# stijnherfst/BrickMap

Hardware: AMD Instinct MI355X
Metric: Mrays/sec (primary x spp x bounces) at 1080p 4-bounce (higher is better)
Workload: dtype f32

## Files before the change

### brickmap_amd/csrc/device_types.h

```cpp
#pragma once
#include <cstddef>
#include <cstdint>

#if defined(__HIPCC__)
#define BM_VHD __host__ __device__ inline
#else
#define BM_VHD inline
#endif

namespace bm {

constexpr uint32_t kIndexBits = 0x00000FFFu;
constexpr uint32_t kLoadedBit = 0x80000000u;

BM_VHD uint32_t supercell_of(int sg_xy, int sg_xy2, int cx, int cy, int cz) {
	return static_cast<uint32_t>((cx >> 4) + (cy >> 4) * sg_xy + (cz >> 4) * sg_xy2);
}
BM_VHD size_t index_word_at(int sg_xy, int sg_xy2, int cx, int cy, int cz) {
	return static_cast<size_t>(supercell_of(sg_xy, sg_xy2, cx, cy, cz)) * 4096 + (cx & 15) + (cy & 15) * 16 + (cz & 15) * 256;
}
BM_VHD uint32_t cell_local_index(int cx, int cy, int cz) { return static_cast<uint32_t>(index_word_at(0, 0, cx & 15, cy & 15, cz & 15)); }
BM_VHD size_t brick_first_word(uint32_t pool_base_value, uint32_t index_word) {
	return (static_cast<size_t>(pool_base_value) + (index_word & kIndexBits)) << 4;
}
// ... 6 lines not shown
	int cf_shift;
	uint32_t cf_pxy;
	uint32_t cf_plane;
	uint32_t cf_magic;
	int cf_magic_shift;
	int* load_queue;
	uint32_t* load_queue_count;
	uint32_t queue_cap;
	int cells, cells_height;
	int sg_xy, sg_xy2;
	float grid_size_f, grid_height_f;
	int lod_distance_8x8x8, lod_distance_2x2x2;
	const uint32_t* escape;
};

struct PoolMove {
	uint32_t src, dst, count, supercell;
};

struct RegionDims {
	int lo[3], hi[3], org[3];
	int c0[3], nc[3], g0;
	uint32_t sg_xy, sg_xy2;
	int64_t row_pitch, slice_pitch;
};

struct LabelDims {
	int lo[3], hi[3], org[3];
	uint32_t nx, ny, nz;
	int c0[3], nc[3];
	uint32_t sg_xy, sg_xy2;
};

struct FrameConstants {
	float right[3], up[3], dir[3], origin[3];
	int campos[3];
	float focal3;
	float lens_radius;
	float sun_direction[3];
	float sun_angular_cos;
	float cone_extent;
	float cone_dir[3], cone_o1[3], cone_o2[3];
	float sunE;
	float rayleigh[3];
	float mie[3];
	float inv_total[3];
	float mixf;
	int width, height;
	int spp, sample_base, max_bounces;
	uint32_t base_frame;
	uint32_t flags;
	int band_rows, shard_rank, shard_count, local_rows;
	int tiles_x, tiles_y;
	int xcd_handout;
	int refill_min;
	uint32_t div_samples_magic, div_tiles_x_magic, div_band_magic, div_st_x_magic;
	int div_samples_shift, div_tiles_x_shift, div_band_shift, div_st_x_shift;
	int helpers;
	uint32_t shadow_field_off;
	uint32_t view_field_off;
	float* accum;
	uint32_t* dbg;
	int frames_after;
	int ring_uniform;
	int ring_sample_stride;
	uint32_t ring_pixel_stride;
	int ring_group;
	int ring_groups_after;
};

struct DeviceCounters {
	unsigned long long v[8];
	unsigned long long sched[8];
	unsigned long long cycles[8];
	unsigned long long detail[8];
};

struct WfRay {
	float origin[3], direction[3], throughput[3], normal[3];
	float distance;
	int identifier;
	int bounces;
	uint32_t pixel_index;
};
static_assert(sizeof(WfRay) == 64, "RayQueue is 64 bytes");

struct WfShadow {
	float origin[3], direction[3], color[3];
	uint32_t pixel_index;
};
static_assert(sizeof(WfShadow) == 40, "ShadowQueue is 40 bytes");

struct WfState {
	uint32_t primary_ray_cnt;
	uint32_t shadow_ray_cnt;
	uint32_t start_position;
	uint32_t generated;
	uint32_t last_survivors, last_shadow;
	uint32_t reserved[26];
	uint32_t extend_ticket[32];
	uint32_t connect_ticket[32];
};
// ... 4 lines not shown
```

### brickmap_amd/csrc/trace.hip

```cpp
#include <type_traits>

#include "kernels.h"
#include "traverse.h"

namespace bm {

__device__ __forceinline__ uint32_t div_const(uint32_t n, uint32_t magic, int shift) { return magic ? (__umulhi(n, magic) >> shift) : n; }

typedef float bm_v4f __attribute__((ext_vector_type(4)));
typedef __attribute__((address_space(1))) bm_v4f v4f_in_global_memory;
typedef __attribute__((address_space(1))) uint32_t u32_in_global_memory;
__device__ __forceinline__ float4 pixel_load(const float4* p) { const bm_v4f v = *(const v4f_in_global_memory*)p; return make_float4(v.x, v.y, v.z, v.w); }
__device__ __forceinline__ void pixel_store(float4* p, float4 v) { const bm_v4f w = {v.x, v.y, v.z, v.w}; *(v4f_in_global_memory*)p = w; }
__device__ __forceinline__ void record_atomic_add(uint32_t* p, uint32_t v) { (void)__hip_atomic_fetch_add((u32_in_global_memory*)p, v, __ATOMIC_RELAXED, __HIP_MEMORY_SCOPE_AGENT); }

__device__ __forceinline__ void pixel_atomic_add(float* p, float v) {
	typedef __attribute__((address_space(1))) float float_in_global_memory;
	[[clang::atomic(ignore_denormal_mode)]] { (void)__hip_atomic_fetch_add((float_in_global_memory*)p, v, __ATOMIC_RELAXED, __HIP_MEMORY_SCOPE_AGENT); }
}

enum : int { P_GEN = 0, P_EXT_DONE = 1, P_SHD_DONE = 2, P_SHD_LAST = 3, P_HELPER = 6, P_SETUP = 8,
             P_SETUP_EXT = P_SETUP | P_EXT_DONE,
             P_SETUP_SHD = P_SETUP | P_SHD_DONE,
             P_SETUP_SHD_LAST = P_SETUP | P_SHD_LAST,
             P_SETUP_HELP = P_SETUP | P_HELPER };
enum : int { ST_IDLE = 4, ST_CONN = 5 };

#ifndef BM_WAVES_PER_SIMD
#define BM_WAVES_PER_SIMD 7
#endif
#ifndef BM_ITEM_LANES
#define BM_ITEM_LANES 1
#endif
#ifndef BM_PRIO
#define BM_PRIO 1
#endif
#ifndef BM_PRIO_A
#define BM_PRIO_A 1
#endif
#ifndef BM_PRIO_B
// ... 65 lines not shown
	Tally tally;
	HitInfo info;
	uint32_t d0 = 0, d1 = 0, d2 = 0xFFFFFFFFu, d3 = 0, hseg = 2166136261u, hsh = 2166136261u, next = 0, nsh = 0, loads0 = 0;
	const bool ray_digest = DBG && (fg.flags & 32u) != 0u;
	uint32_t ray_key = 0, ray_loads0 = 0;

	RayState r;
	constexpr bool kEscape = BM_ESCAPE != 0 && !DBG && (BM_ESCAPE_XCD != 0 || !XCD);
	constexpr bool kSun = BM_SUNFIELD != 0 && kEscape && (BM_SUNFIELD_XCD != 0 || !XCD);
	constexpr bool kShade = BM_SHADOWHEIGHT != 0 && kSun && !DBG && (BM_SHADOWHEIGHT_XCD != 0 || !XCD);
	constexpr bool kView = BM_VIEWFIELD != 0 && kEscape && !DBG && (BM_VIEWFIELD_XCD != 0 || !XCD);
	uint32_t esc = 0;
	r.hit = false;
	r.n = mk(0.f, 0.f, 0.f);
	int state = ST_IDLE;
	int pstate = P_GEN;
	int s = 0;
	int s_end = 0;
	int bounces = 0;
	f3 hitp = mk(0.f, 0.f, 0.f);
	f3 pn = mk(0.f, 0.f, 0.f);
	f3 scolor = mk(0.f, 0.f, 0.f);
	f3 bdir = mk(0.f, 0.f, 0.f);
	float4 acc = make_float4(0.f, 0.f, 0.f, 0.f);
	auto add_rgb = [&](f3 c) {
		if (HELP) { float* a = reinterpret_cast<float*>(accum + local_pixel); pixel_atomic_add(a + 0, c.x); pixel_atomic_add(a + 1, c.y); pixel_atomic_add(a + 2, c.z); }
		else { acc.x += c.x; acc.y += c.y; acc.z += c.z; }
	};
	auto add_terminated = [&]() {
		if (HELP) pixel_atomic_add(reinterpret_cast<float*>(accum + local_pixel) + 3, 1.f);
		else acc.w += 1.f;
	};

	typename std::conditional<RING == 1, int, bool>::type work_left = 1;
	constexpr uint32_t kCounters = XCD ? 8u : BM_WORK_COUNTERS, kCounterStride = 32;
	constexpr uint32_t kXcdTiles = 16u, kStChunks = kXcdTiles * kXcdTiles * 16u;
	constexpr bool xcd_handout = XCD;
	auto first_counter = [&]() {
		return xcd_handout ? static_cast<int>(blockIdx.x % kCounters)
						   : static_cast<int>((blockIdx.x * 4u + static_cast<uint32_t>(__builtin_amdgcn_readfirstlane(static_cast<int>(threadIdx.x >> 6)))) % kCounters);
	};
	int my_counter = first_counter();
	int counters_done = 0;
	auto round_budget = [&]() {
		const long long budget = (static_cast<long long>(total_chunks) + 64) * (static_cast<long long>(fg.spp) + 1) * (fg.max_bounces + 2) *
								 (2ll * sc.cells + sc.cells_height + 64) * (kRing ? fg.frames_after + 1 : 1);
		return static_cast<long long>((static_cast<unsigned long long>(static_cast<uint32_t>(__builtin_amdgcn_readfirstlane(static_cast<int>(budget >> 32)))) << 32) |
									  static_cast<uint32_t>(__builtin_amdgcn_readfirstlane(static_cast<int>(budget))));
	};
	long long rounds_left = round_budget();
	uint32_t runsA = 0, lanesA = 0, runsB = 0, lanesB = 0, runsC = 0, lanesC = 0, runsD = 0, lanesD = 0, runsJ = 0, lanesJ = 0;

	unsigned long long cycA = 0, cycB = 0, cycC = 0, cycD = 0;
	unsigned long long det[8] = {0, 0, 0, 0, 0, 0, 0, 0};
#ifdef BM_PHASE_TIMING
#define BM_MARK(k, tprev) do { const unsigned long long bm_now_ = __builtin_amdgcn_s_memtime(); det[k] += bm_now_ - tprev; tprev = bm_now_; } while (0)
#else
#define BM_MARK(k, tprev) do { } while (0)
#endif
	const unsigned long long t_begin = BM_TIMED ? __builtin_amdgcn_s_memtime() : 0ull;
	unsigned long long t_dry = 0ull;

	for (;;) {
		BM_REGION("refill");
		const unsigned long long idle = __ballot(state == ST_IDLE);
		const int nI = __popcll(idle);
		if (RING == 1 && work_left == 2 && nI == 64) {
			++ring_pos;
			accum = reinterpret_cast<float4*>(fc.accum);
			if (DBG) dbg = fc.dbg;
			work_left = 1;
		}
		if (work_left == 1 && nI >= fg.refill_min) {
			const int want = nI / BM_ITEM_LANES;
			uint32_t base = 0;
			if (lane == 0) base = atomicAdd(work_counter + (kRing ? static_cast<uint32_t>(ring_pos) * static_cast<uint32_t>(kWorkCounterBytes / sizeof(uint32_t)) : 0u) + my_counter * kCounterStride, static_cast<uint32_t>(want));
			base = __builtin_amdgcn_readfirstlane(base);
			const uint32_t st_x = (static_cast<uint32_t>(fg.tiles_x) + kXcdTiles - 1u) / kXcdTiles, st_y = (static_cast<uint32_t>(fg.tiles_y) + kXcdTiles - 1u) / kXcdTiles;
			const uint32_t total_units = xcd_handout ? st_x * st_y : (total_chunks + 3u) >> 2;
			const uint32_t my_units = total_units > static_cast<uint32_t>(my_counter)
										  ? (total_units - static_cast<uint32_t>(my_counter) + kCounters - 1u) / kCounters : 0u;
			const uint32_t my_tickets = my_units * (xcd_handout ? kStChunks : 4u) * items_per_chunk;
			const uint32_t counter_now = static_cast<uint32_t>(my_counter);
			const int ring_at_refill = kRing ? ring_pos : 0;
			if (kRing && !XCD && base + want >= my_tickets && more_frames()) {
				if (kUniform) ++ring_pos;
				else work_left = 2;
			} else if (base + want >= my_tickets) {
				my_counter = (my_counter + 1) % static_cast<int>(kCounters);
				if (++counters_done >= static_cast<int>(kCounters)) {
					if (kRing && more_frames()) {
						counters_done = 0;
						my_counter = first_counter();
						if (kUniform) ++ring_pos;
						else work_left = 2;
					} else {
						work_left = 0;
						if (BM_TIMED) t_dry = __builtin_amdgcn_s_memtime();
					}
				}
			}
			const int rank = __builtin_amdgcn_mbcnt_hi(static_cast<uint32_t>(idle >> 32), __builtin_amdgcn_mbcnt_lo(static_cast<uint32_t>(idle), 0u));
			if (state == ST_IDLE && rank < want * BM_ITEM_LANES) {
				const uint32_t item = base + static_cast<uint32_t>(rank / BM_ITEM_LANES);
				static_assert((kParts & (kParts - 1u)) == 0u, "kParts is a power of two");
				const uint32_t ticket = div_const(item / kParts, fg.div_samples_magic, fg.div_samples_shift), item_sub = item - ticket * items_per_chunk;
				uint32_t item_sample = item_sub / kParts;
				const uint32_t part = item_sub % kParts;
				int item_frame = ring_at_refill;
				if (kUniform) {
					const int group = fg.ring_group;
					item_frame *= group;
					if (group > 1) { item_frame += static_cast<int>(item_sample); item_sample = 0u; }
				}
				uint32_t k;
				int tile_x, tile_y;
				bool in_frame;
				if (xcd_handout) {
					const uint32_t st = (ticket / kStChunks) * kCounters + counter_now, in_st = ticket % kStChunks;
					const uint32_t tw = in_st >> 4;
					k = in_st & 15u;
					const uint32_t st_row = div_const(st, fg.div_st_x_magic, fg.div_st_x_shift);
					tile_x = static_cast<int>((st - st_row * st_x) * kXcdTiles + tw % kXcdTiles);
					tile_y = static_cast<int>(st_row * kXcdTiles + tw / kXcdTiles);
					in_frame = tile_x < fg.tiles_x && tile_y < fg.tiles_y;
				} else {
					const uint32_t chunk = ((ticket >> 2) * kCounters + counter_now) * 4u + (ticket & 3u);
					const uint32_t tile = chunk >> 4;
					k = chunk & 15u;
					tile_y = static_cast<int>(div_const(tile, fg.div_tiles_x_magic, fg.div_tiles_x_shift));
					tile_x = static_cast<int>(tile - static_cast<uint32_t>(tile_y) * static_cast<uint32_t>(fg.tiles_x));
					in_frame = chunk < total_chunks;
				}
				if (kUniform) in_frame = in_frame && item_frame <= fg.frames_after;
				if (item < my_tickets && in_frame) {
					const int cx = static_cast<int>((k & 1u) | ((k >> 1) & 2u)), cy = static_cast<int>(((k >> 1) & 1u) | ((k >> 2) & 2u));
					const uint32_t q = part * BM_ITEM_LANES + (static_cast<uint32_t>(rank) % BM_ITEM_LANES);
					const int x = tile_x * 16 + cx * 4 + static_cast<int>(q & 3u);
					const int ly = tile_y * 16 + cy * 4 + static_cast<int>(q >> 2);
					const int band = static_cast<int>(div_const(static_cast<uint32_t>(ly), fg.div_band_magic, fg.div_band_shift));
					const int y = (band * fg.shard_count + fg.shard_rank) * fg.band_rows + (ly - band * fg.band_rows);
					if (x < fg.width && ly < fg.local_rows && y < fg.height) {
						p = static_cast<uint32_t>(y) * W + static_cast<uint32_t>(x);
						local_pixel = static_cast<uint32_t>(ly) * W + static_cast<uint32_t>(x);
						xy = static_cast<uint32_t>(x) | (static_cast<uint32_t>(y) << 16);
						s = sample_items ? static_cast<int>(item_sample) : 0;
						s_end = sample_items ? s + 1 : fg.spp;
						if (kUniform) {
							const int sample_off = __mul24(item_frame, fg.ring_sample_stride);
							s += sample_off; s_end += sample_off;
							local_pixel += static_cast<uint32_t>(item_frame) * fg.ring_pixel_stride;
						}
						pstate = P_GEN;
						state = ST_NEED;
						if (!HELP) acc = atomic_acc ? make_float4(0.f, 0.f, 0.f, 0.f) : pixel_load(accum + local_pixel);
						if (DBG) {
							d0 = 0; d1 = 0; d2 = 0xFFFFFFFFu; d3 = 0; hseg = 2166136261u; hsh = 2166136261u; next = 0; nsh = 0;
							loads0 = tally.index_loads;
						}
					}
				}
			}
		}
		BM_REGION("policy");
		const int nJ = __popcll(__ballot(state == ST_JUMP));
		const int nA = __popcll(__ballot(state == ST_OUTER)) + nJ;
		const int nB = __popcll(__ballot(state == ST_CAND));
		const int nC = __popcll(__ballot(state == ST_NEED) | __ballot(state == ST_CONN));
		const int live = nA + nB + nC;
		--rounds_left;
		if (rounds_left < 0 || (live == 0 && work_left == 0)) break;
		const int quorum = (live * BM_QUORUM_NUM + BM_QUORUM_DIV - 1) / BM_QUORUM_DIV;
		const int quorum_shade = (live * BM_QUORUM_SHADE_NUM + BM_QUORUM_SHADE_DIV - 1) / BM_QUORUM_SHADE_DIV;
		int phase;
		if (nC >= quorum_shade) phase = 2;
		else if (nB >= quorum) phase = 1;
		else if (nA > 0) phase = 0;
		else phase = nC >= nB ? 2 : 1;

		const unsigned long long t_phase = BM_TIMED ? __builtin_amdgcn_s_memtime() : 0ull;
		if (phase == 2) {
			if (BM_PRIO) __builtin_amdgcn_s_setprio(BM_PRIO_C);
			if (BM_TIMED) {
				const int n_conn = __popcll(__ballot(state == ST_CONN));
				runsC++; lanesC += nC - n_conn;
				if (n_conn) { runsD++; lanesD += n_conn; }
			}
			unsigned long long t_sub = t_phase;
			(void)t_sub;
			BM_REGION("C.connect");
			if (state == ST_NEED || state == ST_CONN) {
				if (state == ST_CONN) {
					const bool occluded = r.hit;
					if (DBG) {
						tally.shadow_rays++;
						nsh++;
						hsh = hmix(hsh, static_cast<uint32_t>(occluded));
						if (occluded) {
							hsh = hmix(hsh, static_cast<uint32_t>(info.brick_id));
							hsh = hmix(hsh, static_cast<uint32_t>(info.sub_id) | (static_cast<uint32_t>(info.level) << 12));
						}
						if (ray_digest && dbg) {
							uint32_t e = hmix(hmix(2166136261u, ray_key), static_cast<uint32_t>(occluded));
							if (occluded) {
								e = hmix(e, static_cast<uint32_t>(info.brick_id));
								e = hmix(e, static_cast<uint32_t>(info.sub_id) | (static_cast<uint32_t>(info.level) << 12));
							}
							uint32_t* d = dbg + static_cast<size_t>(local_pixel) * 8;
							record_atomic_add(d + 5, e); record_atomic_add(d + 6, 1u << 16); record_atomic_add(d + 7, tally.index_loads - ray_loads0);
						}
					}
					if (HELP && pstate == P_HELPER) {
						if (!occluded) {
							float* a = reinterpret_cast<float*>(accum + local_pixel);
							pixel_atomic_add(a + 0, scolor.x); pixel_atomic_add(a + 1, scolor.y); pixel_atomic_add(a + 2, scolor.z);
						}
						state = ST_IDLE;
					} else {
						if (!occluded) {
							add_rgb(scolor);
						}
						state = ST_NEED;
						if (pstate == P_SHD_LAST) {
							s++;
							pstate = P_GEN;
						} else {
							bounces++;
							pstate = P_SETUP_EXT;
						}
					}
				}
				BM_MARK(0, t_sub);
				BM_REGION("C.shade");
				if (pstate == P_EXT_DONE) {
					const bool is_hit = r.hit;
					pn = r.n;
					if (DBG) {
						tally.extend_rays++;
						next++;
						if (s == 0 && bounces == 0) {
							d0 = is_hit ? __float_as_uint(r.distance) : 0u;
							d1 = is_hit ? (pack_normal(pn) | (1u << 8) | (static_cast<uint32_t>(info.level) << 12)) : 0u;
							d2 = is_hit ? static_cast<uint32_t>(info.brick_id) : 0xFFFFFFFFu;
							d3 = is_hit ? static_cast<uint32_t>(info.sub_id) : 0u;
						}
						hseg = hmix(hseg, static_cast<uint32_t>(is_hit));
						if (is_hit) {
							hseg = hmix(hseg, __float_as_uint(r.distance));
							hseg = hmix(hseg, pack_normal(pn) | (static_cast<uint32_t>(info.level) << 12));
							hseg = hmix(hseg, static_cast<uint32_t>(info.brick_id));
							hseg = hmix(hseg, static_cast<uint32_t>(info.sub_id));
						}
						if (ray_digest && dbg) {
							uint32_t e = hmix(hmix(2166136261u, ray_key), static_cast<uint32_t>(is_hit));
							if (is_hit) {
								e = hmix(e, __float_as_uint(r.distance));
								e = hmix(e, pack_normal(pn) | (static_cast<uint32_t>(info.level) << 12));
								e = hmix(e, static_cast<uint32_t>(info.brick_id));
								e = hmix(e, static_cast<uint32_t>(info.sub_id));
							}
							uint32_t* d = dbg + static_cast<size_t>(local_pixel) * 8;
							record_atomic_add(d + 4, e); record_atomic_add(d + 6, 1u); record_atomic_add(d + 7, tally.index_loads - ray_loads0);
							if (ray_key == 0u) {
								u32_in_global_memory* g = (u32_in_global_memory*)d;
								g[0] = d0; g[1] = d1; g[2] = d2; g[3] = d3;
							}
						}
					}
					const bool primary_only = fg.flags & 1u;
					float sunLight = 0.f;
					bool cast = false;
					if (is_hit && !primary_only) {
						hitp = hitp + r.d * r.distance;
						hitp = hitp + pn * 2.f * kEpsilon;
						uint32_t sh_cell = 0u, sh_entry = 0u;
						if (kShade) {
							const uint32_t plane = fc.shadow_field_off;
							const ShadowOrigin so = shadow_origin(sc.grid_size_f, sc.grid_height_f, sc.cells, sc.cells_height, sc.cf_shift, sc.cf_pxy, plane, hitp.x, hitp.y, hitp.z);
							sh_cell = plane != 0u ? so.cell : kShadowUndecided;
							sh_entry = sc.escape[so.entry];
						}
						const uint32_t frame = fc.base_frame + static_cast<uint32_t>(bounces);
						const uint32_t slot = p + static_cast<uint32_t>(fc.sample_base + s) * W * H;
						uint32_t sseed = (frame * p * 147565741u) * 720898027u * slot;
						r.d = cone_sample(fc, sseed);
						sunLight = dot(pn, r.d);
						cast = sunLight > 0.f;
						const bool terminated = !(bounces < fg.max_bounces);
						if (terminated) {
							add_terminated();
						} else {
							bdir = bounce_direction(pn, sseed);
						}
						if (kShade) cast = cast && !(sh_cell < sh_entry);
						if (cast) pstate = terminated ? P_SETUP_SHD_LAST : P_SETUP_SHD;
						else if (terminated) { s++; pstate = P_GEN; }
						else { bounces++; pstate = P_SETUP_EXT; }
					}
					BM_MARK(1, t_sub);
					BM_REGION("C.sky");
					if (!is_hit || cast) {
						const SkyView sv = sky_view(fc, r.d);
						if (cast) {
							scolor = (sun_from_view(fc, sv) * sunLight) * 1E-5f;
						} else {
							f3 c;
							if (bounces == 0) c = fc.sun_angular_cos == 1.0f ? mk(1.0f, 0.0f, 0.0f) : sunsky_from_view(fc, sv);
							else c = sky_from_view(fc, sv);
							add_rgb(c);
						}
					}
					if (!is_hit || primary_only) {
						add_terminated();
						s++;
						pstate = P_GEN;
					}
				}
				BM_MARK(2, t_sub);
			}
			BM_REGION("C.hand-over");
			if (HELP) {
				static_assert((P_SETUP_SHD | 1) == P_SETUP_SHD_LAST, "the two states of a shadow ray drawn in this pass differ in bit 0");
				const bool hand = (pstate | 1) == P_SETUP_SHD_LAST;
				const unsigned long long hand_m = __ballot(hand), free_m = __ballot(state == ST_IDLE);
				if (hand_m != 0ull && free_m != 0ull) {
					const int n_pairs = min(__popcll(hand_m), __popcll(free_m));
					const int hrank = __builtin_amdgcn_mbcnt_hi(static_cast<uint32_t>(hand_m >> 32), __builtin_amdgcn_mbcnt_lo(static_cast<uint32_t>(hand_m), 0u));
					const int frank = __builtin_amdgcn_mbcnt_hi(static_cast<uint32_t>(free_m >> 32), __builtin_amdgcn_mbcnt_lo(static_cast<uint32_t>(free_m), 0u));
					const bool gives = hand && hrank < n_pairs, takes = state == ST_IDLE && frank < n_pairs;
					if (gives) {
						const uint32_t k = static_cast<uint32_t>(hrank);
						staging_word(lds_brick, k, 0) = hitp.x; staging_word(lds_brick, k, 1) = hitp.y; staging_word(lds_brick, k, 2) = hitp.z;
						staging_word(lds_brick, k, 3) = r.d.x; staging_word(lds_brick, k, 4) = r.d.y; staging_word(lds_brick, k, 5) = r.d.z;
						staging_word(lds_brick, k, 6) = scolor.x; staging_word(lds_brick, k, 7) = scolor.y; staging_word(lds_brick, k, 8) = scolor.z;
						staging_word(lds_brick, k, 9) = __uint_as_float(local_pixel);
						if (DBG) staging_word(lds_brick, k, 10) = __uint_as_float((static_cast<uint32_t>(s) << 8) | static_cast<uint32_t>(bounces));
						if (pstate == P_SETUP_SHD_LAST) { s++; pstate = P_GEN; }
						else { bounces++; pstate = P_SETUP_EXT; }
					}
					__builtin_amdgcn_fence(__ATOMIC_RELEASE, "wavefront");
					__builtin_amdgcn_wave_barrier();
// ... 3 lines not shown
						hitp = mk(staging_word(lds_brick, k, 0), staging_word(lds_brick, k, 1), staging_word(lds_brick, k, 2));
						r.d = mk(staging_word(lds_brick, k, 3), staging_word(lds_brick, k, 4), staging_word(lds_brick, k, 5));
						scolor = mk(staging_word(lds_brick, k, 6), staging_word(lds_brick, k, 7), staging_word(lds_brick, k, 8));
						local_pixel = __float_as_uint(staging_word(lds_brick, k, 9));
						if (DBG) ray_key = __float_as_uint(staging_word(lds_brick, k, 10));
						pstate = P_SETUP_HELP;
					}
				}
			}
			BM_REGION("C.generate");
			if (state == ST_NEED) {
				if (pstate == P_GEN) {
					if (s >= s_end) {
						if (HELP) {
						} else if (atomic_acc) {
							float* a = reinterpret_cast<float*>(accum + local_pixel);
							pixel_atomic_add(a + 0, acc.x); pixel_atomic_add(a + 1, acc.y); pixel_atomic_add(a + 2, acc.z); pixel_atomic_add(a + 3, acc.w);
						} else {
							pixel_store(accum + local_pixel, acc);
						}
						if (DBG && dbg && !ray_digest) {
							u32_in_global_memory* d = (u32_in_global_memory*)(dbg + static_cast<size_t>(local_pixel) * 8);
							if (sample_items) {
								if (s_end == 1) { d[0] = d0; d[1] = d1; d[2] = d2; d[3] = d3; }
								record_atomic_add((uint32_t*)(d + 4), hseg); record_atomic_add((uint32_t*)(d + 5), hsh); record_atomic_add((uint32_t*)(d + 6), next | (nsh << 16));
								record_atomic_add((uint32_t*)(d + 7), tally.index_loads - loads0);
							} else {
								d[0] = d0; d[1] = d1; d[2] = d2; d[3] = d3; d[4] = hseg; d[5] = hsh; d[6] = next | (nsh << 16);
								d[7] = tally.index_loads - loads0;
							}
						}
						state = ST_IDLE;
					} else {
						const uint32_t slot = p + static_cast<uint32_t>(fc.sample_base + s) * W * H;
						uint32_t seed = (fc.base_frame * 147565741u) * 720898027u * slot;
						primary_ray(fc, seed, xy & 0xFFFFu, xy >> 16, hitp, bdir);
						pn = mk(0.f, 0.f, 0.f);
						bounces = 0;
						if (DBG) tally.paths++;
						pstate = P_SETUP_EXT;
					}
				}
				BM_MARK(3, t_sub);
			}
			BM_REGION("C.set-up");
			if (pstate >= P_SETUP) {
				pstate &= P_SETUP - 1;
				const bool shadow = pstate != P_EXT_DONE;
				r.n = shadow ? mk(0.f, 0.f, 0.f) : pn;
				if (DBG) {
					if (!(HELP && pstate == P_HELPER)) ray_key = (static_cast<uint32_t>(s) << 8) | static_cast<uint32_t>(bounces);
					ray_loads0 = tally.index_loads;
				}
				const f3 dir = shadow ? r.d : bdir;
				const int st = ray_setup<DBG, kEscape, kView, true>(sc, hitp, dir, r, tally, &esc, kSun && shadow ? fc.shadow_field_off : 0u,
															  kView && !shadow && bounces == 0 ? fc.view_field_off : 0u);
				state = (st == ST_NEED && shadow) ? ST_CONN : st;
			}
			BM_MARK(4, t_sub);
		} else if (phase == 1) {
			BM_REGION("B.candidate");
			if (BM_PRIO) __builtin_amdgcn_s_setprio(BM_PRIO_B);
			if (BM_TIMED) { runsB++; lanesB += nB; }
#ifdef BM_SHARE_PROBE
			{
				const bool cand = state == ST_CAND;
				const uint32_t cell_id = r.p - r.field_off;
				bool dup = false;
				for (int l = 0; l < 63; ++l) {
					const uint32_t other = static_cast<uint32_t>(__builtin_amdgcn_readlane(static_cast<int>(cell_id), l));
					const bool other_cand = (__ballot(cand) >> l) & 1ull;
					dup = dup || (cand && other_cand && lane > l && other == cell_id);
				}
				const int n_dup = __popcll(__ballot(dup));
				if (__ballot(cand) != 0ull) { det[5] += 1; det[6] += n_dup ? 1 : 0; det[7] += static_cast<unsigned long long>(n_dup); }
			}
#endif
#ifdef BM_PHASE_TIMING
			uint32_t walk_trips = 0;
			if (state == ST_CAND) {
				int st = process_candidate<DBG>(sc, fc.campos, r, info, tally, lds_brick, &walk_trips);
#else
			if (state == ST_CAND) {
				int st = process_candidate<DBG>(sc, fc.campos, r, info, tally, lds_brick);
#endif
				state = (st == ST_NEED && pstate != P_EXT_DONE) ? ST_CONN : st;
			}
#if defined(BM_PHASE_TIMING) && !defined(BM_SHARE_PROBE)
			{
// ... 189 lines not shown
```

### brickmap_amd/csrc/traverse.h

```cpp
#pragma once
#include <hip/hip_runtime.h>

#include "detmath.h"
#include "device_types.h"
#include "escape.h"
#include "jump.h"
#include "steps.h"

namespace bm {

namespace {

constexpr float kPi = 3.1415926535897932f;
constexpr float kEpsilon = 0.001f;
constexpr uint32_t kLodBits = 0xFF000u;
constexpr uint32_t kUnloadedBit = 0x40000000u;
constexpr uint32_t kRequestedBit = 0x20000000u;

struct f3 {
	float x, y, z;
};
__device__ __forceinline__ f3 mk(float x, float y, float z) { return f3{x, y, z}; }
__device__ __forceinline__ f3 operator+(f3 a, f3 b) { return mk(a.x + b.x, a.y + b.y, a.z + b.z); }
__device__ __forceinline__ f3 operator-(f3 a, f3 b) { return mk(a.x - b.x, a.y - b.y, a.z - b.z); }
// ... 391 lines not shown
		if (intersect_grid<8, DBG>(o8, r.d, sx, sy, sz, r.dx, r.dy, r.dz, r.n, sub_distance, brick, 0u, sub, tally, lds_brick, walk_trips, reinterpret_cast<const uint32_t*>(bq))) {
			r.distance = new_distance * 8.f + sub_distance + r.tminn;
			if (INFO) { info.level = 2; info.sub_id = sub; }
			r.hit = true;
			return ST_NEED;
		}
	} else if (index & kUnloadedBit) {
		const uint32_t old = REQUEST ? atomicOr(&sc.index_grid[flat], kRequestedBit) : kRequestedBit;
		if (!(old & kRequestedBit)) {
			const uint32_t load_index = atomicAdd(sc.load_queue_count, 1u);
			if (load_index < sc.queue_cap) {
				int* q = sc.load_queue + 3 * static_cast<size_t>(load_index);
				q[0] = px; q[1] = py; q[2] = pz;
				if (DBG) tally.requests++;
			} else {
				atomicAnd(&sc.index_grid[flat], ~kRequestedBit);
			}
		}
		r.distance = new_distance * 8.f + r.tminn;
		if (INFO) { info.level = 3; info.sub_id = 0; }
		r.hit = true;
		return ST_NEED;
	}
	return ST_OUTER;
}

__device__ __forceinline__ float fast_div(float a, float b) { return a * __builtin_amdgcn_rcpf(b); }
__device__ __forceinline__ float fast_sqrt(float a) { return __builtin_amdgcn_sqrtf(a); }
__device__ __forceinline__ float fast_exp(float a) { return __expf(a); }
struct SkyView {
	f3 Fex;
	float cosViewSun;
};
__device__ __forceinline__ SkyView sky_view(const FrameConstants& fc, f3 viewDir) {
	SkyView o;
	o.cosViewSun = dot(viewDir, ld3(fc.sun_direction));
	const float cosUpView = dot(mk(0.f, 0.f, 1.f), viewDir);
	const float zenith = gmax(0.0f, cosUpView);
	const float inv_zenith = __builtin_amdgcn_rcpf(zenith);
	const float rayleighLen = 8.4E3f * inv_zenith;
	const float mieLen = 1.25E3f * inv_zenith;
	const f3 a = ld3(fc.rayleigh) * rayleighLen + ld3(fc.mie) * mieLen;
	o.Fex = mk(fast_exp(-a.x), fast_exp(-a.y), fast_exp(-a.z));
	return o;
}
__device__ __forceinline__ f3 sky_scatter(const FrameConstants& fc, const SkyView& v) {
	const float c = v.cosViewSun;
	const float rayleighPhase = (3.0f / (16.0f * kPi)) * (1.0f + c * c);
	const float g = 0.80f, g2 = 0.80f * 0.80f;
	const float base = 1.0f - 2.0f * g * c + g2;
	const float hg = (1.0f / (4.0f * kPi)) * fast_div(1.0f - g2, base * fast_sqrt(base));
	const f3 light = ld3(fc.rayleigh) * rayleighPhase + ld3(fc.mie) * hg;
	const f3 somethingElse = mk(light.x * fc.inv_total[0], light.y * fc.inv_total[1], light.z * fc.inv_total[2]) * fc.sunE;
	const f3 sky = somethingElse * mk(1.0f - v.Fex.x, 1.0f - v.Fex.y, 1.0f - v.Fex.z);
	const f3 q = somethingElse * v.Fex;
	const f3 p = mk(fast_sqrt(q.x), fast_sqrt(q.y), fast_sqrt(q.z));
	const float a = fc.mixf;
	return sky * mk(1.0f * (1.0f - a) + p.x * a, 1.0f * (1.0f - a) + p.y * a, 1.0f * (1.0f - a) + p.z * a);
}
__device__ __forceinline__ f3 sun_from_view(const FrameConstants& fc, const SkyView& v) {
	const float sundisk = static_cast<double>(fc.sun_angular_cos) < (v.cosViewSun != 0.0f ? 1.0 : 0.0) ? 1.0f : 0.0f;
	return ((v.Fex * (fc.sunE * 19000.0f)) * sundisk) * 0.01f;
}
__device__ __forceinline__ f3 sky_from_view(const FrameConstants& fc, const SkyView& v) {
	return sky_scatter(fc, v) * (1.f * 0.01f);
}
__device__ __forceinline__ f3 sunsky_from_view(const FrameConstants& fc, const SkyView& v) {
	const f3 sky = sky_scatter(fc, v);
	const float e0 = fc.sun_angular_cos, e1 = fc.sun_angular_cos + 0.00002f;
	const float s = gmin(gmax(fast_div(v.cosViewSun - e0, e1 - e0), 0.0f), 1.0f);
	const float sundisk = s * s * (3.0f - 2.0f * s);
	const f3 sun = ((v.Fex * (fc.sunE * 19000.0f)) * sundisk) * 1E-5f;
	return (sun + sky) * 0.01f;
}
__device__ __forceinline__ f3 sun_radiance(const FrameConstants& fc, f3 viewDir) { return sun_from_view(fc, sky_view(fc, viewDir)); }
__device__ __forceinline__ f3 sky_radiance(const FrameConstants& fc, f3 viewDir) { return sky_from_view(fc, sky_view(fc, viewDir)); }
__device__ __forceinline__ f3 sunsky_radiance(const FrameConstants& fc, f3 viewDir) {
	if (fc.sun_angular_cos == 1.0f) return mk(1.0f, 0.0f, 0.0f);
	return sunsky_from_view(fc, sky_view(fc, viewDir));
}

__device__ __forceinline__ f3 cone_sample(const FrameConstants& fc, uint32_t& seed) {
	const f3 dir = ld3(fc.cone_dir), o1 = ld3(fc.cone_o1), o2 = ld3(fc.cone_o2);
	float rx = random_float2(seed);
	float ry = random_float2(seed);
	rx = rx * 2.f * kPi;
	ry = 1.0f - ry * fc.cone_extent;
	const float oneminus = sqrtf(1.0f - ry * ry);
	float s, c;
	det_sincos(rx, s, c);
	return (o1 * (c * oneminus) + o2 * (s * oneminus)) + dir * ry;
}

__device__ __forceinline__ void primary_ray(const FrameConstants& fc, uint32_t seed, uint32_t x, uint32_t y, f3& origin, f3& direction) {
	const f3 cam_right = ld3(fc.right), cam_up = ld3(fc.up), cam_dir = ld3(fc.dir), cam_o = ld3(fc.origin);
	const float W = static_cast<float>(static_cast<uint32_t>(fc.width)), H = static_cast<float>(static_cast<uint32_t>(fc.height));
	const int stratum = static_cast<int>(random_float(seed) * (16 + 0.99999f));
	const int stratumX = stratum % 4, stratumY = (stratum / 4) % 4;
	const float jx = 0.25f * stratumX + (random_float(seed) * 0.25f);
	const float jy = 0.25f * stratumY + (random_float(seed) * 0.25f);
	const float ppx = static_cast<float>(x) - jx;
	const float ppy = static_cast<float>(y) - jy;
	const float ni = (ppx / W) - 0.5f;
	const float nj = ((H - ppy) / H) - 0.5f;
	const f3 to_focal = normalize(cam_dir + cam_right * ni + cam_up * nj);
	const f3 convergence = cam_o + to_focal * fc.focal3;
	origin = cam_o;
	if (fc.lens_radius != 0.f) {
		const float l0 = random_float(seed);
		const float l1 = random_float(seed);
		float lx = 0.f, ly = 0.f;
		const float ox = 2.f * l0 - 1.f, oy = 2.f * l1 - 1.f;
		if (!(ox == 0 && oy == 0)) {
			float theta, rr;
			if (fabsf(ox) > fabsf(oy)) { rr = ox; theta = kPi / 4 * (oy / ox); }
			else { rr = oy; theta = kPi / 2 - kPi / 4 * (ox / oy); }
			float sn, cs;
			det_sincos(theta, sn, cs);
			lx = rr * cs;
			ly = rr * sn;
		}
		const float plx = fc.lens_radius * lx, ply = fc.lens_radius * ly;
		origin = cam_o + cam_right * plx + cam_up * ply;
	}
	direction = normalize(convergence - origin);
}

// ... 34 lines not shown
```

Measured before the change: 15870.

## Regroup frame constants into contiguous runs and load them as wide vectors

```diff
diff --git a/brickmap_amd/csrc/device_types.h b/brickmap_amd/csrc/device_types.h
--- a/brickmap_amd/csrc/device_types.h
+++ b/brickmap_amd/csrc/device_types.h
@@ -62,42 +62,52 @@
 	uint32_t sg_xy, sg_xy2;
 };
 
-struct FrameConstants {
+struct alignas(64) FrameConstants {
 	float right[3], up[3], dir[3], origin[3];
-	int campos[3];
 	float focal3;
 	float lens_radius;
+	int campos[3];
+	float cone_dir[3], cone_o1[3], cone_o2[3];
+	float cone_extent;
 	float sun_direction[3];
 	float sun_angular_cos;
-	float cone_extent;
-	float cone_dir[3], cone_o1[3], cone_o2[3];
 	float sunE;
 	float rayleigh[3];
 	float mie[3];
 	float inv_total[3];
 	float mixf;
-	int width, height;
-	int spp, sample_base, max_bounces;
+	int width;
+	int sample_base;
 	uint32_t base_frame;
+	int max_bounces;
 	uint32_t flags;
-	int band_rows, shard_rank, shard_count, local_rows;
-	int tiles_x, tiles_y;
-	int xcd_handout;
-	int refill_min;
-	uint32_t div_samples_magic, div_tiles_x_magic, div_band_magic, div_st_x_magic;
-	int div_samples_shift, div_tiles_x_shift, div_band_shift, div_st_x_shift;
 	int helpers;
 	uint32_t shadow_field_off;
 	uint32_t view_field_off;
 	float* accum;
 	uint32_t* dbg;
+	int xcd_handout;
+	int refill_min;
+	int ring_uniform;
+	int ring_groups_after;
+	int reserved_[2];
+	uint32_t div_st_x_magic; int div_st_x_shift;
+	int height;
 	int frames_after;
-	int ring_uniform;
+	int tiles_x, tiles_y;
+	uint32_t div_samples_magic; int div_samples_shift;
+	uint32_t div_tiles_x_magic; int div_tiles_x_shift;
+	uint32_t div_band_magic; int div_band_shift;
+	int band_rows, shard_rank, shard_count, local_rows;
+	int spp;
+	int ring_group;
 	int ring_sample_stride;
 	uint32_t ring_pixel_stride;
-	int ring_group;
-	int ring_groups_after;
 };
+static_assert(sizeof(FrameConstants) == 320 && offsetof(FrameConstants, div_st_x_magic) == 240 && offsetof(FrameConstants, tiles_x) == 256 &&
+              offsetof(FrameConstants, ring_pixel_stride) == 316, "the hand-out block: four words, then one cache line of sixteen (trace.hip Handout)");
+static_assert(offsetof(FrameConstants, view_field_off) == offsetof(FrameConstants, shadow_field_off) + 4 && offsetof(FrameConstants, shadow_field_off) % 8 == 0,
+              "the two plane offsets are read as a pair (trace.hip set-up)");
 
 struct DeviceCounters {
 	unsigned long long v[8];
diff --git a/brickmap_amd/csrc/trace.hip b/brickmap_amd/csrc/trace.hip
--- a/brickmap_amd/csrc/trace.hip
+++ b/brickmap_amd/csrc/trace.hip
@@ -5,7 +5,83 @@
 
 namespace bm {
 
-__device__ __forceinline__ uint32_t div_const(uint32_t n, uint32_t magic, int shift) { return magic ? (__umulhi(n, magic) >> shift) : n; }
+__device__ __forceinline__ uint32_t div_const(uint32_t n, uint32_t magic, int shift) {
+	const uint32_t q = __umulhi(n, magic) >> shift;
+	return magic ? q : n;
+}
+
+struct Handout {
+	uint32_t div_st_x_magic; int div_st_x_shift;
+	int height, frames_after, tiles_x, tiles_y;
+	uint32_t div_samples_magic; int div_samples_shift;
+	uint32_t div_tiles_x_magic; int div_tiles_x_shift;
+	uint32_t div_band_magic; int div_band_shift;
+	int band_rows, shard_rank, shard_count, local_rows, spp, ring_group, ring_sample_stride;
+	uint32_t ring_pixel_stride;
+};
+typedef uint32_t bm_v2u __attribute__((ext_vector_type(2)));
+typedef uint32_t bm_v4u __attribute__((ext_vector_type(4)));
+typedef uint32_t bm_v8u __attribute__((ext_vector_type(8)));
+typedef uint32_t bm_v16u __attribute__((ext_vector_type(16)));
+
+struct FrameWords { int width, sample_base; uint32_t base_frame; int max_bounces; uint32_t flags; int helpers; uint32_t shadow_field_off, view_field_off; };
+struct ConeWords { float cone_dir[3], cone_o1[3], cone_o2[3]; float cone_extent; };
+struct SkyWords { float cone_extent; float sun_direction[3]; float sun_angular_cos, sunE; float rayleigh[3], mie[3], inv_total[3]; float mixf; };
+struct CameraWords { float right[3], up[3], dir[3], origin[3]; float focal3, lens_radius; };
+struct GenerateWords { int width, sample_base; uint32_t base_frame; int max_bounces; };
+struct PrimaryConsts : CameraWords { int width, height; };
+#define BM_RUN_OF(T, first, last) (offsetof(FrameConstants, last) - offsetof(FrameConstants, first) == offsetof(T, last))
+static_assert(BM_RUN_OF(FrameWords, width, sample_base) && BM_RUN_OF(FrameWords, width, base_frame) && BM_RUN_OF(FrameWords, width, max_bounces) && BM_RUN_OF(FrameWords, width, flags) &&
+              BM_RUN_OF(FrameWords, width, helpers) && BM_RUN_OF(FrameWords, width, shadow_field_off) && BM_RUN_OF(FrameWords, width, view_field_off), "FrameWords");
+static_assert(BM_RUN_OF(ConeWords, cone_dir, cone_o1) && BM_RUN_OF(ConeWords, cone_dir, cone_o2) && BM_RUN_OF(ConeWords, cone_dir, cone_extent), "ConeWords");
+static_assert(BM_RUN_OF(SkyWords, cone_extent, sun_direction) && BM_RUN_OF(SkyWords, cone_extent, sun_angular_cos) && BM_RUN_OF(SkyWords, cone_extent, sunE) &&
+              BM_RUN_OF(SkyWords, cone_extent, rayleigh) && BM_RUN_OF(SkyWords, cone_extent, mie) && BM_RUN_OF(SkyWords, cone_extent, inv_total) && BM_RUN_OF(SkyWords, cone_extent, mixf), "SkyWords");
+static_assert(BM_RUN_OF(CameraWords, right, up) && BM_RUN_OF(CameraWords, right, dir) && BM_RUN_OF(CameraWords, right, origin) && BM_RUN_OF(CameraWords, right, focal3) &&
+              BM_RUN_OF(CameraWords, right, lens_radius), "CameraWords");
+#undef BM_RUN_OF
+template <class T>
+__device__ __forceinline__ T load_words(const void* first) {
+	typedef bm_v16u v16 __attribute__((aligned(4))); typedef bm_v8u v8 __attribute__((aligned(4))); typedef bm_v4u v4 __attribute__((aligned(4))); typedef bm_v2u v2 __attribute__((aligned(4)));
+	constexpr int N = sizeof(T) / 4;
+	static_assert(sizeof(T) % 4 == 0 && std::is_trivially_copyable<T>::value, "a run of words");
+	const uint32_t* p = static_cast<const uint32_t*>(first);
+	uint32_t w[N];
+	constexpr int n16 = N / 16 * 16, n8 = n16 + (N - n16) / 8 * 8, n4 = n8 + (N - n8) / 4 * 4, n2 = n4 + (N - n4) / 2 * 2;
+#pragma unroll
+	for (int i = 0; i < n16; i += 16) { const bm_v16u v = *reinterpret_cast<const v16*>(p + i); for (int k = 0; k < 16; ++k) w[i + k] = v[k]; }
+#pragma unroll
+	for (int i = n16; i < n8; i += 8) { const bm_v8u v = *reinterpret_cast<const v8*>(p + i); for (int k = 0; k < 8; ++k) w[i + k] = v[k]; }
+#pragma unroll
+	for (int i = n8; i < n4; i += 4) { const bm_v4u v = *reinterpret_cast<const v4*>(p + i); for (int k = 0; k < 4; ++k) w[i + k] = v[k]; }
+#pragma unroll
+	for (int i = n4; i < n2; i += 2) { const bm_v2u v = *reinterpret_cast<const v2*>(p + i); for (int k = 0; k < 2; ++k) w[i + k] = v[k]; }
+	if (n2 < N) w[n2] = p[n2];
+	T t;
+	__builtin_memcpy(&t, w, sizeof t);
+	return t;
+}
+template <bool BLOCK>
+__device__ __forceinline__ decltype(auto) sky_terms(const FrameConstants& fc) {
+	if constexpr (BLOCK) return load_words<SkyWords>(&fc.cone_extent);
+	else return (fc);
+}
+__device__ __forceinline__ Handout load_handout(const FrameConstants& fg) {
+	static_assert(offsetof(FrameConstants, height) == offsetof(FrameConstants, div_st_x_magic) + 8 && offsetof(FrameConstants, tiles_x) == offsetof(FrameConstants, div_st_x_magic) + 16 &&
+	              offsetof(FrameConstants, div_samples_magic) == offsetof(FrameConstants, tiles_x) + 8 && offsetof(FrameConstants, div_band_shift) == offsetof(FrameConstants, tiles_x) + 28 &&
+	              offsetof(FrameConstants, band_rows) == offsetof(FrameConstants, tiles_x) + 32 && offsetof(FrameConstants, spp) == offsetof(FrameConstants, tiles_x) + 48 &&
+	              offsetof(FrameConstants, ring_pixel_stride) == offsetof(FrameConstants, tiles_x) + 60, "the hand-out block's words, in Handout's order");
+	const bm_v4u a = *reinterpret_cast<const bm_v4u*>(&fg.div_st_x_magic);
+	const bm_v16u b = *reinterpret_cast<const bm_v16u*>(&fg.tiles_x);
+	Handout h;
+	h.div_st_x_magic = a[0]; h.div_st_x_shift = static_cast<int>(a[1]); h.height = static_cast<int>(a[2]); h.frames_after = static_cast<int>(a[3]);
+	h.tiles_x = static_cast<int>(b[0]); h.tiles_y = static_cast<int>(b[1]);
+	h.div_samples_magic = b[2]; h.div_samples_shift = static_cast<int>(b[3]);
+	h.div_tiles_x_magic = b[4]; h.div_tiles_x_shift = static_cast<int>(b[5]);
+	h.div_band_magic = b[6]; h.div_band_shift = static_cast<int>(b[7]);
+	h.band_rows = static_cast<int>(b[8]); h.shard_rank = static_cast<int>(b[9]); h.shard_count = static_cast<int>(b[10]); h.local_rows = static_cast<int>(b[11]);
+	h.spp = static_cast<int>(b[12]); h.ring_group = static_cast<int>(b[13]); h.ring_sample_stride = static_cast<int>(b[14]); h.ring_pixel_stride = b[15];
+	return h;
+}
 
 typedef float bm_v4f __attribute__((ext_vector_type(4)));
 typedef __attribute__((address_space(1))) bm_v4f v4f_in_global_memory;
@@ -137,7 +213,8 @@
 		else acc.w += 1.f;
 	};
 
-	typename std::conditional<RING == 1, int, bool>::type work_left = 1;
+	constexpr int kNoRefill = 65, kFrameDone = 0x100;
+	int refill_at = fg.refill_min;
 	constexpr uint32_t kCounters = XCD ? 8u : BM_WORK_COUNTERS, kCounterStride = 32;
 	constexpr uint32_t kXcdTiles = 16u, kStChunks = kXcdTiles * kXcdTiles * 16u;
 	constexpr bool xcd_handout = XCD;
@@ -170,18 +247,20 @@
 		BM_REGION("refill");
 		const unsigned long long idle = __ballot(state == ST_IDLE);
 		const int nI = __popcll(idle);
-		if (RING == 1 && work_left == 2 && nI == 64) {
-			++ring_pos;
-			accum = reinterpret_cast<float4*>(fc.accum);
-			if (DBG) dbg = fc.dbg;
-			work_left = 1;
-		}
-		if (work_left == 1 && nI >= fg.refill_min) {
+		if (nI >= refill_at) {
+			if (RING == 1 && (counters_done & kFrameDone)) {
+				++ring_pos;
+				accum = reinterpret_cast<float4*>(fc.accum);
+				if (DBG) dbg = fc.dbg;
+				counters_done &= ~kFrameDone;
+				refill_at = fg.refill_min;
+			}
+			const Handout ho = load_handout(fg);
 			const int want = nI / BM_ITEM_LANES;
 			uint32_t base = 0;
 			if (lane == 0) base = atomicAdd(work_counter + (kRing ? static_cast<uint32_t>(ring_pos) * static_cast<uint32_t>(kWorkCounterBytes / sizeof(uint32_t)) : 0u) + my_counter * kCounterStride, static_cast<uint32_t>(want));
 			base = __builtin_amdgcn_readfirstlane(base);
-			const uint32_t st_x = (static_cast<uint32_t>(fg.tiles_x) + kXcdTiles - 1u) / kXcdTiles, st_y = (static_cast<uint32_t>(fg.tiles_y) + kXcdTiles - 1u) / kXcdTiles;
+			const uint32_t st_x = (static_cast<uint32_t>(ho.tiles_x) + kXcdTiles - 1u) / kXcdTiles, st_y = (static_cast<uint32_t>(ho.tiles_y) + kXcdTiles - 1u) / kXcdTiles;
 			const uint32_t total_units = xcd_handout ? st_x * st_y : (total_chunks + 3u) >> 2;
 			const uint32_t my_units = total_units > static_cast<uint32_t>(my_counter)
 										  ? (total_units - static_cast<uint32_t>(my_counter) + kCounters - 1u) / kCounters : 0u;
@@ -190,7 +269,7 @@
 			const int ring_at_refill = kRing ? ring_pos : 0;
 			if (kRing && !XCD && base + want >= my_tickets && more_frames()) {
 				if (kUniform) ++ring_pos;
-				else work_left = 2;
+				else { counters_done |= kFrameDone; refill_at = 64; }
 			} else if (base + want >= my_tickets) {
 				my_counter = (my_counter + 1) % static_cast<int>(kCounters);
 				if (++counters_done >= static_cast<int>(kCounters)) {
@@ -198,9 +277,9 @@
 						counters_done = 0;
 						my_counter = first_counter();
 						if (kUniform) ++ring_pos;
-						else work_left = 2;
+						else { counters_done = kFrameDone; refill_at = 64; }
 					} else {
-						work_left = 0;
+						refill_at = kNoRefill;
 						if (BM_TIMED) t_dry = __builtin_amdgcn_s_memtime();
 					}
 				}
@@ -209,12 +288,12 @@
 			if (state == ST_IDLE && rank < want * BM_ITEM_LANES) {
 				const uint32_t item = base + static_cast<uint32_t>(rank / BM_ITEM_LANES);
 				static_assert((kParts & (kParts - 1u)) == 0u, "kParts is a power of two");
-				const uint32_t ticket = div_const(item / kParts, fg.div_samples_magic, fg.div_samples_shift), item_sub = item - ticket * items_per_chunk;
+				const uint32_t ticket = div_const(item / kParts, ho.div_samples_magic, ho.div_samples_shift), item_sub = item - ticket * items_per_chunk;
 				uint32_t item_sample = item_sub / kParts;
 				const uint32_t part = item_sub % kParts;
 				int item_frame = ring_at_refill;
 				if (kUniform) {
-					const int group = fg.ring_group;
+					const int group = ho.ring_group;
 					item_frame *= group;
 					if (group > 1) { item_frame += static_cast<int>(item_sample); item_sample = 0u; }
 				}
@@ -225,36 +304,36 @@
 					const uint32_t st = (ticket / kStChunks) * kCounters + counter_now, in_st = ticket % kStChunks;
 					const uint32_t tw = in_st >> 4;
 					k = in_st & 15u;
-					const uint32_t st_row = div_const(st, fg.div_st_x_magic, fg.div_st_x_shift);
+					const uint32_t st_row = div_const(st, ho.div_st_x_magic, ho.div_st_x_shift);
 					tile_x = static_cast<int>((st - st_row * st_x) * kXcdTiles + tw % kXcdTiles);
 					tile_y = static_cast<int>(st_row * kXcdTiles + tw / kXcdTiles);
-					in_frame = tile_x < fg.tiles_x && tile_y < fg.tiles_y;
+					in_frame = tile_x < ho.tiles_x && tile_y < ho.tiles_y;
 				} else {
 					const uint32_t chunk = ((ticket >> 2) * kCounters + counter_now) * 4u + (ticket & 3u);
 					const uint32_t tile = chunk >> 4;
 					k = chunk & 15u;
-					tile_y = static_cast<int>(div_const(tile, fg.div_tiles_x_magic, fg.div_tiles_x_shift));
-					tile_x = static_cast<int>(tile - static_cast<uint32_t>(tile_y) * static_cast<uint32_t>(fg.tiles_x));
+					tile_y = static_cast<int>(div_const(tile, ho.div_tiles_x_magic, ho.div_tiles_x_shift));
+					tile_x = static_cast<int>(tile - static_cast<uint32_t>(tile_y) * static_cast<uint32_t>(ho.tiles_x));
 					in_frame = chunk < total_chunks;
 				}
-				if (kUniform) in_frame = in_frame && item_frame <= fg.frames_after;
+				if (kUniform) in_frame = in_frame && item_frame <= ho.frames_after;
 				if (item < my_tickets && in_frame) {
 					const int cx = static_cast<int>((k & 1u) | ((k >> 1) & 2u)), cy = static_cast<int>(((k >> 1) & 1u) | ((k >> 2) & 2u));
 					const uint32_t q = part * BM_ITEM_LANES + (static_cast<uint32_t>(rank) % BM_ITEM_LANES);
 					const int x = tile_x * 16 + cx * 4 + static_cast<int>(q & 3u);
 					const int ly = tile_y * 16 + cy * 4 + static_cast<int>(q >> 2);
-					const int band = static_cast<int>(div_const(static_cast<uint32_t>(ly), fg.div_band_magic, fg.div_band_shift));
-					const int y = (band * fg.shard_count + fg.shard_rank) * fg.band_rows + (ly - band * fg.band_rows);
-					if (x < fg.width && ly < fg.local_rows && y < fg.height) {
+					const int band = static_cast<int>(div_const(static_cast<uint32_t>(ly), ho.div_band_magic, ho.div_band_shift));
+					const int y = (band * ho.shard_count + ho.shard_rank) * ho.band_rows + (ly - band * ho.band_rows);
+					if (static_cast<uint32_t>(x) < W && ly < ho.local_rows && y < ho.height) {
 						p = static_cast<uint32_t>(y) * W + static_cast<uint32_t>(x);
 						local_pixel = static_cast<uint32_t>(ly) * W + static_cast<uint32_t>(x);
 						xy = static_cast<uint32_t>(x) | (static_cast<uint32_t>(y) << 16);
 						s = sample_items ? static_cast<int>(item_sample) : 0;
-						s_end = sample_items ? s + 1 : fg.spp;
+						s_end = sample_items ? s + 1 : ho.spp;
 						if (kUniform) {
-							const int sample_off = __mul24(item_frame, fg.ring_sample_stride);
+							const int sample_off = __mul24(item_frame, ho.ring_sample_stride);
 							s += sample_off; s_end += sample_off;
-							local_pixel += static_cast<uint32_t>(item_frame) * fg.ring_pixel_stride;
+							local_pixel += static_cast<uint32_t>(item_frame) * ho.ring_pixel_stride;
 						}
 						pstate = P_GEN;
 						state = ST_NEED;
@@ -274,7 +353,7 @@
 		const int nC = __popcll(__ballot(state == ST_NEED) | __ballot(state == ST_CONN));
 		const int live = nA + nB + nC;
 		--rounds_left;
-		if (rounds_left < 0 || (live == 0 && work_left == 0)) break;
+		if (rounds_left < 0 || (live == 0 && refill_at == kNoRefill)) break;
 		const int quorum = (live * BM_QUORUM_NUM + BM_QUORUM_DIV - 1) / BM_QUORUM_DIV;
 		const int quorum_shade = (live * BM_QUORUM_SHADE_NUM + BM_QUORUM_SHADE_DIV - 1) / BM_QUORUM_SHADE_DIV;
 		int phase;
@@ -338,6 +417,8 @@
 				BM_MARK(0, t_sub);
 				BM_REGION("C.shade");
 				if (pstate == P_EXT_DONE) {
+					const FrameWords kc = load_words<FrameWords>(&fc.width);
+					const ConeWords kcone = load_words<ConeWords>(&fc.cone_dir);
 					const bool is_hit = r.hit;
 					pn = r.n;
 					if (DBG) {
@@ -372,7 +453,7 @@
 							}
 						}
 					}
-					const bool primary_only = fg.flags & 1u;
+					const bool primary_only = kc.flags & 1u;
 					float sunLight = 0.f;
 					bool cast = false;
 					if (is_hit && !primary_only) {
@@ -380,18 +461,18 @@
 						hitp = hitp + pn * 2.f * kEpsilon;
 						uint32_t sh_cell = 0u, sh_entry = 0u;
 						if (kShade) {
-							const uint32_t plane = fc.shadow_field_off;
+							const uint32_t plane = kc.shadow_field_off;
 							const ShadowOrigin so = shadow_origin(sc.grid_size_f, sc.grid_height_f, sc.cells, sc.cells_height, sc.cf_shift, sc.cf_pxy, plane, hitp.x, hitp.y, hitp.z);
 							sh_cell = plane != 0u ? so.cell : kShadowUndecided;
 							sh_entry = sc.escape[so.entry];
 						}
-						const uint32_t frame = fc.base_frame + static_cast<uint32_t>(bounces);
-						const uint32_t slot = p + static_cast<uint32_t>(fc.sample_base + s) * W * H;
+						const uint32_t frame = kc.base_frame + static_cast<uint32_t>(bounces);
+						const uint32_t slot = p + static_cast<uint32_t>(kc.sample_base + s) * W * H;
 						uint32_t sseed = (frame * p * 147565741u) * 720898027u * slot;
-						r.d = cone_sample(fc, sseed);
+						r.d = cone_sample(kcone, sseed);
 						sunLight = dot(pn, r.d);
 						cast = sunLight > 0.f;
-						const bool terminated = !(bounces < fg.max_bounces);
+						const bool terminated = !(bounces < kc.max_bounces);
 						if (terminated) {
 							add_terminated();
 						} else {
@@ -405,13 +486,14 @@
 					BM_MARK(1, t_sub);
 					BM_REGION("C.sky");
 					if (!is_hit || cast) {
-						const SkyView sv = sky_view(fc, r.d);
+						const auto& ks = sky_terms<HELP>(fc);
+						const SkyView sv = sky_view(ks, r.d);
 						if (cast) {
-							scolor = (sun_from_view(fc, sv) * sunLight) * 1E-5f;
+							scolor = (sun_from_view(ks, sv) * sunLight) * 1E-5f;
 						} else {
 							f3 c;
-							if (bounces == 0) c = fc.sun_angular_cos == 1.0f ? mk(1.0f, 0.0f, 0.0f) : sunsky_from_view(fc, sv);
-							else c = sky_from_view(fc, sv);
+							if (bounces == 0) c = ks.sun_angular_cos == 1.0f ? mk(1.0f, 0.0f, 0.0f) : sunsky_from_view(ks, sv);
+							else c = sky_from_view(ks, sv);
 							add_rgb(c);
 						}
 					}
@@ -481,9 +563,13 @@
 						}
 						state = ST_IDLE;
 					} else {
-						const uint32_t slot = p + static_cast<uint32_t>(fc.sample_base + s) * W * H;
-						uint32_t seed = (fc.base_frame * 147565741u) * 720898027u * slot;
-						primary_ray(fc, seed, xy & 0xFFFFu, xy >> 16, hitp, bdir);
+						const GenerateWords kg = load_words<GenerateWords>(&fc.width);
+						PrimaryConsts kcam;
+						static_cast<CameraWords&>(kcam) = load_words<CameraWords>(&fc.right);
+						kcam.width = kg.width; kcam.height = fg.height;
+						const uint32_t slot = p + static_cast<uint32_t>(kg.sample_base + s) * W * H;
+						uint32_t seed = (kg.base_frame * 147565741u) * 720898027u * slot;
+						primary_ray(kcam, seed, xy & 0xFFFFu, xy >> 16, hitp, bdir);
 						pn = mk(0.f, 0.f, 0.f);
 						bounces = 0;
 						if (DBG) tally.paths++;
@@ -502,8 +588,10 @@
 					ray_loads0 = tally.index_loads;
 				}
 				const f3 dir = shadow ? r.d : bdir;
-				const int st = ray_setup<DBG, kEscape, kView, true>(sc, hitp, dir, r, tally, &esc, kSun && shadow ? fc.shadow_field_off : 0u,
-															  kView && !shadow && bounces == 0 ? fc.view_field_off : 0u);
+				const bm_v2u planes = kSun || kView ? *reinterpret_cast<const bm_v2u*>(&fc.shadow_field_off) : bm_v2u{0u, 0u};
+				const uint32_t sun_plane = planes[0], view_plane = planes[1];
+				const int st = ray_setup<DBG, kEscape, kView, true>(sc, hitp, dir, r, tally, &esc, kSun && shadow ? sun_plane : 0u,
+															  kView && !shadow && bounces == 0 ? view_plane : 0u);
 				state = (st == ST_NEED && shadow) ? ST_CONN : st;
 			}
 			BM_MARK(4, t_sub);
diff --git a/brickmap_amd/csrc/traverse.h b/brickmap_amd/csrc/traverse.h
--- a/brickmap_amd/csrc/traverse.h
+++ b/brickmap_amd/csrc/traverse.h
@@ -447,7 +447,8 @@
 	f3 Fex;
 	float cosViewSun;
 };
-__device__ __forceinline__ SkyView sky_view(const FrameConstants& fc, f3 viewDir) {
+template <class C>
+__device__ __forceinline__ SkyView sky_view(const C& fc, f3 viewDir) {
 	SkyView o;
 	o.cosViewSun = dot(viewDir, ld3(fc.sun_direction));
 	const float cosUpView = dot(mk(0.f, 0.f, 1.f), viewDir);
@@ -459,7 +460,8 @@
 	o.Fex = mk(fast_exp(-a.x), fast_exp(-a.y), fast_exp(-a.z));
 	return o;
 }
-__device__ __forceinline__ f3 sky_scatter(const FrameConstants& fc, const SkyView& v) {
+template <class C>
+__device__ __forceinline__ f3 sky_scatter(const C& fc, const SkyView& v) {
 	const float c = v.cosViewSun;
 	const float rayleighPhase = (3.0f / (16.0f * kPi)) * (1.0f + c * c);
 	const float g = 0.80f, g2 = 0.80f * 0.80f;
@@ -473,14 +475,17 @@
 	const float a = fc.mixf;
 	return sky * mk(1.0f * (1.0f - a) + p.x * a, 1.0f * (1.0f - a) + p.y * a, 1.0f * (1.0f - a) + p.z * a);
 }
-__device__ __forceinline__ f3 sun_from_view(const FrameConstants& fc, const SkyView& v) {
+template <class C>
+__device__ __forceinline__ f3 sun_from_view(const C& fc, const SkyView& v) {
 	const float sundisk = static_cast<double>(fc.sun_angular_cos) < (v.cosViewSun != 0.0f ? 1.0 : 0.0) ? 1.0f : 0.0f;
 	return ((v.Fex * (fc.sunE * 19000.0f)) * sundisk) * 0.01f;
 }
-__device__ __forceinline__ f3 sky_from_view(const FrameConstants& fc, const SkyView& v) {
+template <class C>
+__device__ __forceinline__ f3 sky_from_view(const C& fc, const SkyView& v) {
 	return sky_scatter(fc, v) * (1.f * 0.01f);
 }
-__device__ __forceinline__ f3 sunsky_from_view(const FrameConstants& fc, const SkyView& v) {
+template <class C>
+__device__ __forceinline__ f3 sunsky_from_view(const C& fc, const SkyView& v) {
 	const f3 sky = sky_scatter(fc, v);
 	const float e0 = fc.sun_angular_cos, e1 = fc.sun_angular_cos + 0.00002f;
 	const float s = gmin(gmax(fast_div(v.cosViewSun - e0, e1 - e0), 0.0f), 1.0f);
@@ -495,7 +500,8 @@
 	return sunsky_from_view(fc, sky_view(fc, viewDir));
 }
 
-__device__ __forceinline__ f3 cone_sample(const FrameConstants& fc, uint32_t& seed) {
+template <class C>
+__device__ __forceinline__ f3 cone_sample(const C& fc, uint32_t& seed) {
 	const f3 dir = ld3(fc.cone_dir), o1 = ld3(fc.cone_o1), o2 = ld3(fc.cone_o2);
 	float rx = random_float2(seed);
 	float ry = random_float2(seed);
@@ -507,7 +513,8 @@
 	return (o1 * (c * oneminus) + o2 * (s * oneminus)) + dir * ry;
 }
 
-__device__ __forceinline__ void primary_ray(const FrameConstants& fc, uint32_t seed, uint32_t x, uint32_t y, f3& origin, f3& direction) {
+template <class C>
+__device__ __forceinline__ void primary_ray(const C& fc, uint32_t seed, uint32_t x, uint32_t y, f3& origin, f3& direction) {
 	const f3 cam_right = ld3(fc.right), cam_up = ld3(fc.up), cam_dir = ld3(fc.dir), cam_o = ld3(fc.origin);
 	const float W = static_cast<float>(static_cast<uint32_t>(fc.width)), H = static_cast<float>(static_cast<uint32_t>(fc.height));
 	const int stratum = static_cast<int>(random_float(seed) * (16 + 0.99999f));
```

Result: no change. 15990, median of 6 (+0.7%).
